# dragonlong/articulated-pose

Measured on AMD Instinct MI355X. Metric: point-clouds/sec (N=1024, eyeglasses ANCSH infer+pose-fit), higher is better.
Workload: dtype f32 (network) / f64 (joint LM)

## Files before the change

### articulated-pose_amd/csrc/pose.hip

```cpp
#include "common.h"
#include "pose_math.h"

namespace ancsh {
namespace pose {

constexpr int MODEL_A = 13;
constexpr int MODEL_B = 26;

__device__ __forceinline__ unsigned long long splitmix64(unsigned long long x) {
    x += 0x9E3779B97F4A7C15ull;
    x = (x ^ (x >> 30)) * 0xBF58476D1CE4E5B9ull;
    x = (x ^ (x >> 27)) * 0x94D049BB133111EBull;
    return x ^ (x >> 31);
}
__device__ __forceinline__ int device_draw(unsigned long long seed, int prob, int iter, int k, int n) {
    const unsigned long long h = splitmix64(seed ^ splitmix64(((unsigned long long)prob << 40) ^ ((unsigned long long)iter << 8) ^ (unsigned)k));
    return (int)(h % (unsigned long long)n);
}
enum { KEY_VALUE = 0, KEY_DSEED = 1, KEY_DKEY = 2 };
struct DKey {
    const ancsh_stream_key *key;
    int parts;
};
template <int KM> struct KeyArgT { typedef unsigned long long type; };
template <> struct KeyArgT<KEY_DKEY> { typedef DKey type; };
template <int KM> using KeyArg = typename KeyArgT<KM>::type;

template <int KM>
__device__ __forceinline__ unsigned long long kernel_seed(unsigned long long arg, unsigned add) {
    return KM != KEY_VALUE ? *(const unsigned long long *__restrict__)arg + add : arg;
}
template <int KM>
__device__ __forceinline__ unsigned long long kernel_seed(DKey arg, unsigned add) {
    return arg.key->seed + add;
}
template <int KM>
__device__ __forceinline__ int key_problem_base(unsigned long long) { return 0; }
template <int KM>
__device__ __forceinline__ int key_problem_base(DKey arg) { return arg.key->cloud_base * arg.parts; }

__device__ __forceinline__ double wave_sum(double v) {
#pragma unroll
    for (int o = 32; o > 0; o >>= 1) v += __shfl_xor(v, o, 64);
    return v;
}
template <int K>
__device__ __forceinline__ void block_sum(double (&v)[K], double *red, int nwaves) {
    const int lane = threadIdx.x & 63, wave = threadIdx.x >> 6;
#pragma unroll
    for (int i = 0; i < K; ++i) v[i] = wave_sum(v[i]);
    __syncthreads();
    if (lane == 0)
#pragma unroll
        for (int i = 0; i < K; ++i) red[wave * K + i] = v[i];
    __syncthreads();
#pragma unroll
    for (int i = 0; i < K; ++i) {
        double s = 0.0;
        for (int w = 0; w < nwaves; ++w) s += red[w * K + i];
        v[i] = s;
    }
}

__device__ __forceinline__ void estimate_single3(const float s[3][3], const float t[3][3], float R[9], float &scale,
                                                 float tr[3]) {
    double sm[3], tm[3];
#pragma unroll
    for (int c = 0; c < 3; ++c) {
        sm[c] = ((double)s[0][c] + s[1][c] + s[2][c]) / 3.0;
        tm[c] = ((double)t[0][c] + t[1][c] + t[2][c]) / 3.0;
    }
    double M[9] = {0, 0, 0, 0, 0, 0, 0, 0, 0};
#pragma unroll
    for (int i = 0; i < 3; ++i)
#pragma unroll
        for (int a = 0; a < 3; ++a)
#pragma unroll
            for (int b = 0; b < 3; ++b) M[a * 3 + b] += (t[i][a] - tm[a]) * (s[i][b] - sm[b]);
    double q[4], Rd[9];
    horn_quat_fast(M, q);
    quat_to_mat(q, Rd);
    double ab = 0.0, aa = 0.0;
// ... 643 lines not shown
    for (int i = 0; i < 3; ++i)
#pragma unroll
        for (int j = i + 1; j < 3; ++j) {
            double ds = 0.0, dt = 0.0;
#pragma unroll
            for (int c = 0; c < 3; ++c) {
                const double u = (double)s[i][c] - s[j][c], v = (double)t[i][c] - t[j][c];
                ds += u * u;
                dt += v * v;
            }
            ab += 2.0 * sqrt(ds) * sqrt(dt);
            aa += 2.0 * ds;
            bb += 2.0 * dt;
        }
    sc = (float)(ab / (aa + 1e-6));
    sc_inv = (float)(ab / (bb + 1e-6));
}

__device__ __forceinline__ void center_part3(const float s[3][3], const float t[3][3], float sc_inv, double xc[3][3],
                                             double yc[3][3]) {
    float sm[3], tm[3];
#pragma unroll
    for (int c = 0; c < 3; ++c) {
        sm[c] = ((s[0][c] + s[1][c]) + s[2][c]) / 3.0f;
        tm[c] = ((sc_inv * t[0][c] + sc_inv * t[1][c]) + sc_inv * t[2][c]) / 3.0f;
    }
#pragma unroll
    for (int i = 0; i < 3; ++i) {
#pragma unroll
        for (int c = 0; c < 3; ++c) {
            xc[i][c] = (double)(s[i][c] - sm[c]);
            yc[i][c] = (double)(sc_inv * t[i][c] - tm[c]);
        }
    }
}

__device__ __forceinline__ void prep_part3(const float s[3][3], const float t[3][3], float sc_inv, double xc[3][3],
                                           double yc[3][3], double rv[3]) {
    center_part3(s, t, sc_inv, xc, yc);
    double M[9] = {0, 0, 0, 0, 0, 0, 0, 0, 0};
#pragma unroll
    for (int i = 0; i < 3; ++i)
#pragma unroll
        for (int a = 0; a < 3; ++a)
#pragma unroll
            for (int b = 0; b < 3; ++b) M[a * 3 + b] += yc[i][a] * xc[i][b];
    double q[4];
    horn_quat_fast(M, q);
    quat_to_rotvec(q, rv);
}

__device__ __forceinline__ double residual_sq_f64(const double R[9], double sc, const double tr[3], float sx, float sy, float sz,
                                                  float tx, float ty, float tz) {
    const double rx = R[0] * sx + R[1] * sy + R[2] * sz, ry = R[3] * sx + R[4] * sy + R[5] * sz,
                 rz = R[6] * sx + R[7] * sy + R[8] * sz;
    const double ex = ((double)tx - sc * rx) - tr[0], ey = ((double)ty - sc * ry) - tr[1], ez = ((double)tz - sc * rz) - tr[2];
    return ex * ex + ey * ey + ez * ez;
}
__device__ __forceinline__ bool inlier_f64(const double R[9], double sc, const double tr[3], float sx, float sy, float sz,
                                           float tx, float ty, float tz, double th) {
    return residual_sq_f64(R, sc, tr, sx, sy, sz, tx, ty, tz) < th;
}

struct HypSamples {
    float s0[3][3], t0[3][3], s1[3][3], t1[3][3];
};
__device__ __forceinline__ void load_hyp_samples(const float *__restrict__ src, const float *__restrict__ tgt, const int *draws,
                                                 unsigned long long seed, int prob, int kbase, int niter, int h, int a0, int n0, int a1,
                                                 int n1, HypSamples &q) {
    int i0[3], i1[3];
    load_draw3(draws, seed, prob, kbase, niter, h, 0, 6, n0, i0);
    load_draw3(draws, seed, prob, kbase, niter, h, 3, 6, n1, i1);
#pragma unroll
    for (int i = 0; i < 3; ++i)
#pragma unroll
        for (int c = 0; c < 3; ++c) {
            q.s0[i][c] = src[(size_t)(a0 + i0[i]) * 3 + c];
            q.t0[i][c] = tgt[(size_t)(a0 + i0[i]) * 3 + c];
            q.s1[i][c] = src[(size_t)(a1 + i1[i]) * 3 + c];
            q.t1[i][c] = tgt[(size_t)(a1 + i1[i]) * 3 + c];
        }
}

template <int KM>
__global__ __launch_bounds__(64) void ransac_joint_init_kernel(const int *__restrict__ rng0, const int *__restrict__ rng1,
                                                               const float *__restrict__ src, const float *__restrict__ tgt,
                                                               int niter, const int *__restrict__ draws, KeyArg<KM> seed_arg,
                                                               double *__restrict__ scores, double *__restrict__ models) {
    const unsigned long long seed = kernel_seed<KM>(seed_arg, 1);
    const int kbase = key_problem_base<KM>(seed_arg);
    const int prob = blockIdx.y, h = blockIdx.x * 64 + threadIdx.x;
    const int a0 = rng0[prob * 2], n0 = rng0[prob * 2 + 1] - a0;
    const int a1 = rng1[prob * 2], n1 = rng1[prob * 2 + 1] - a1;
    if (h >= niter) return;
    double *mo = models + ((size_t)prob * niter + h) * MODEL_B;
    if (n0 <= 0 || n1 <= 0) {
        scores[(size_t)prob * niter + h] = -1.0;
        for (int i = 0; i < MODEL_B; ++i) mo[i] = NAN;
        return;
    }
    HypSamples q;
    load_hyp_samples(src, tgt, draws, seed, prob, kbase, niter, h, a0, n0, a1, n1, q);
    float sc0, sc0i, sc1, sc1i;
    scales3(q.s0, q.t0, sc0, sc0i);
    scales3(q.s1, q.t1, sc1, sc1i);
    double xc[3][3], yc[3][3], x[6];
    prep_part3(q.s0, q.t0, sc0i, xc, yc, x);
    prep_part3(q.s1, q.t1, sc1i, xc, yc, x + 3);
#pragma unroll
    for (int i = 0; i < 6; ++i) mo[i] = x[i];
    mo[6] = sc0i; mo[7] = sc1i; mo[8] = sc0; mo[9] = sc1;
}

constexpr int HYP_CHUNK = 256;
constexpr int HYP_CHUNK_SMALL = 64;
constexpr long HYP_SMALL_LAUNCH = 8192;
constexpr int HYP_REFILL = 16;

template <int KM, bool PRISM>
__device__ __forceinline__ void ransac_joint_lm_run(const int *__restrict__ rng0, const int *__restrict__ rng1,
                                                    const float *__restrict__ src, const float *__restrict__ tgt,
                                                    const float *__restrict__ joint_dir, int niter,
                                                    const int *__restrict__ draws, KeyArg<KM> seed_arg,
                                                    double *__restrict__ models, int *__restrict__ lm_stat, int chunk) {
    const unsigned long long seed = kernel_seed<KM>(seed_arg, 1);
    const int kbase = key_problem_base<KM>(seed_arg);
    const int prob = blockIdx.y;
    const int a0 = rng0[prob * 2], n0 = rng0[prob * 2 + 1] - a0;
    const int a1 = rng1[prob * 2], n1 = rng1[prob * 2 + 1] - a1;
    if (n0 <= 0 || n1 <= 0) return;
    const int c1 = min(niter, (int)(blockIdx.x + 1) * chunk);
    int next = blockIdx.x * chunk;
    HypProblemT<PRISM> P;
    if constexpr (!PRISM) {
        P.J[0] = joint_dir[prob * 3]; P.J[1] = joint_dir[prob * 3 + 1]; P.J[2] = joint_dir[prob * 3 + 2];
        P.wj = 3.0;
    }
    Lm6 S;
    bool active = false;
    int h = 0;
    for (;;) {
        const unsigned long long idle = __ballot(!active);
        const int n_idle = __popcll(idle);
        if (next < c1 && (n_idle >= HYP_REFILL || n_idle >= c1 - next || n_idle == 64)) {
            if (!active) {
                const int mine = next + __builtin_amdgcn_mbcnt_hi((unsigned)(idle >> 32), __builtin_amdgcn_mbcnt_lo((unsigned)idle, 0));
                if (mine < c1) {
                    h = mine;
                    const double *mo = models + ((size_t)prob * niter + h) * MODEL_B;
                    HypSamples q;
                    load_hyp_samples(src, tgt, draws, seed, prob, kbase, niter, h, a0, n0, a1, n1, q);
                    center_part3(q.s0, q.t0, (float)mo[6], P.x0, P.y0);
                    center_part3(q.s1, q.t1, (float)mo[7], P.x1, P.y1);
#pragma unroll
                    for (int i = 0; i < 6; ++i) S.x[i] = mo[i];
                    lm6_begin(P, S);
                    active = true;
                }
            }
            next += n_idle;
        } else if (n_idle == 64) {
            break;
        }
        if (active && lm6_trip(P, S, 1e-4, 1e-8, 1e-8, 4200)) {
            double *mo = models + ((size_t)prob * niter + h) * MODEL_B;
#pragma unroll
            for (int i = 0; i < 6; ++i) mo[i] = S.x[i];
#ifdef LM_COUNT
            if (lm_stat) { lm_stat[((size_t)prob * niter + h) * 2] = S.info | (S.trips << 4) | (S.nchol << 17); lm_stat[((size_t)prob * niter + h) * 2 + 1] = S.nfev; }
#else
            if (lm_stat) { lm_stat[((size_t)prob * niter + h) * 2] = S.info; lm_stat[((size_t)prob * niter + h) * 2 + 1] = S.nfev; }
#endif
            active = false;
        }
    }
}

template <int KM>
__global__ __launch_bounds__(64) void ransac_joint_lm_kernel(const int *__restrict__ rng0, const int *__restrict__ rng1,
                                                             const float *__restrict__ src, const float *__restrict__ tgt,
                                                             const float *__restrict__ joint_dir, int niter,
                                                             const int *__restrict__ draws, KeyArg<KM> seed_arg,
                                                             double *__restrict__ models, int *__restrict__ lm_stat, int chunk) {
    ransac_joint_lm_run<KM, false>(rng0, rng1, src, tgt, joint_dir, niter, draws, seed_arg, models, lm_stat, chunk);
}

template <int KM>
__global__ __launch_bounds__(64) void ransac_joint_lm_kind_kernel(const int *__restrict__ rng0, const int *__restrict__ rng1,
                                                                  const float *__restrict__ src, const float *__restrict__ tgt,
                                                                  const float *__restrict__ joint_dir, int niter,
                                                                  const int *__restrict__ draws, KeyArg<KM> seed_arg,
                                                                  double *__restrict__ models, int *__restrict__ lm_stat, int chunk,
                                                                  const int *__restrict__ joint_kind) {
    if (joint_kind[blockIdx.y] != 0) ransac_joint_lm_run<KM, true>(rng0, rng1, src, tgt, joint_dir, niter, draws, seed_arg, models, lm_stat, chunk);
    else ransac_joint_lm_run<KM, false>(rng0, rng1, src, tgt, joint_dir, niter, draws, seed_arg, models, lm_stat, chunk);
}

constexpr int COOP_G = 8;
constexpr int COOP_XCH = 112;
constexpr int COOP_HYP_PER_WAVE = 32;

__device__ __forceinline__ void group_lds_fence() {
    __builtin_amdgcn_fence(__ATOMIC_RELEASE, "wavefront");
    __builtin_amdgcn_wave_barrier();
    __builtin_amdgcn_fence(__ATOMIC_ACQUIRE, "wavefront");
}

template <bool PRISM>
struct HypProblemCoopT {
    double x0[3][3], y0[3][3], x1[3][3], y1[3][3], J[3], wj;
    double *xch;
    int role;

    __device__ __forceinline__ double cost(const double x[6]) const {
        const bool joint = role >= 6;
        const bool p1 = role >= 3 && role < 6;
        const int i = joint ? 0 : (p1 ? role - 3 : role);
        double partial;
        if (!joint) {
            const Rod r = p1 ? rod_prepare(x[3], x[4], x[5]) : rod_prepare(x[0], x[1], x[2]);
            const double px = p1 ? (i == 0 ? x1[0][0] : i == 1 ? x1[1][0] : x1[2][0]) : (i == 0 ? x0[0][0] : i == 1 ? x0[1][0] : x0[2][0]);
            const double py = p1 ? (i == 0 ? x1[0][1] : i == 1 ? x1[1][1] : x1[2][1]) : (i == 0 ? x0[0][1] : i == 1 ? x0[1][1] : x0[2][1]);
            const double pz = p1 ? (i == 0 ? x1[0][2] : i == 1 ? x1[1][2] : x1[2][2]) : (i == 0 ? x0[0][2] : i == 1 ? x0[1][2] : x0[2][2]);
            const double tx = p1 ? (i == 0 ? y1[0][0] : i == 1 ? y1[1][0] : y1[2][0]) : (i == 0 ? y0[0][0] : i == 1 ? y0[1][0] : y0[2][0]);
            const double ty = p1 ? (i == 0 ? y1[0][1] : i == 1 ? y1[1][1] : y1[2][1]) : (i == 0 ? y0[0][1] : i == 1 ? y0[1][1] : y0[2][1]);
            const double tz = p1 ? (i == 0 ? y1[0][2] : i == 1 ? y1[1][2] : y1[2][2]) : (i == 0 ? y0[0][2] : i == 1 ? y0[1][2] : y0[2][2]);
            double ox, oy, oz;
            rod_apply(r, px, py, pz, ox, oy, oz);
            const double a = tx - ox, b = ty - oy, c = tz - oz;
            partial = a * a + b * b + c * c;
        } else if constexpr (PRISM) {
            partial = prismatic_cost(x);
        } else {
            const Rod r0 = rod_prepare(x[0], x[1], x[2]), r1 = rod_prepare(x[3], x[4], x[5]);
            double ux, uy, uz, wx, wy, wz;
            rod_apply(r0, J[0], J[1], J[2], ux, uy, uz);
            rod_apply(r1, J[0], J[1], J[2], wx, wy, wz);
            partial = (ux - wx) * (ux - wx) + (uy - wy) * (uy - wy) + (uz - wz) * (uz - wz);
        }
        double *cs = xch + 102;
        if (role < 7) cs[role] = partial;
        group_lds_fence();
        double s = 0.0;
#pragma unroll
        for (int k = 0; k < 3; ++k) { s += cs[k]; s += cs[3 + k]; }
        if constexpr (PRISM) s += cs[6]; else s += wj * cs[6];
        group_lds_fence();
        return s;
    }

    __device__ __forceinline__ void normal(const double x[6], double A[21], double g[6]) const {
        double *col = xch, *jdx = xch + 54, *rhx = xch + 72, *fx = xch + 78, *jux = xch + 96;
        {
            const int cr = role < 6 ? role : role - 6;
            const bool p1 = cr >= 3;
            const int q = p1 ? cr - 3 : cr;
            const double r0 = p1 ? x[3] : x[0], r1 = p1 ? x[4] : x[1], r2 = p1 ? x[5] : x[2];
            const Rod b = rod_prepare(r0, r1, r2);
            const double h = fd_step(q == 0 ? r0 : q == 1 ? r1 : r2);
            const double rh = fast_rcp(h);
            const Rod pr = rod_prepare(r0 + (q == 0 ? h : 0.0), r1 + (q == 1 ? h : 0.0), r2 + (q == 2 ? h : 0.0));
            const bool wr = role < 6;
#pragma unroll
            for (int i = 0; i < 3; ++i) {
                const double px = p1 ? x1[i][0] : x0[i][0], py = p1 ? x1[i][1] : x0[i][1], pz = p1 ? x1[i][2] : x0[i][2];
                const double yx = p1 ? y1[i][0] : y0[i][0], yy = p1 ? y1[i][1] : y0[i][1], yz = p1 ? y1[i][2] : y0[i][2];
                double ox, oy, oz, qx, qy, qz;
                rod_apply(b, px, py, pz, ox, oy, oz);
                const double f0 = yx - ox, f1 = yy - oy, f2 = yz - oz;
                rod_apply(pr, px, py, pz, qx, qy, qz);
                if (wr) {
                    col[cr * 9 + i * 3 + 0] = ((yx - qx) - f0) * rh;
                    col[cr * 9 + i * 3 + 1] = ((yy - qy) - f1) * rh;
                    col[cr * 9 + i * 3 + 2] = ((yz - qz) - f2) * rh;
                    if (q == 0) { fx[(p1 ? 9 : 0) + i * 3] = f0; fx[(p1 ? 9 : 0) + i * 3 + 1] = f1; fx[(p1 ? 9 : 0) + i * 3 + 2] = f2; }
                }
            }
            if constexpr (!PRISM) {
// ... 82 lines not shown
        P.J[0] = joint_dir[prob * 3]; P.J[1] = joint_dir[prob * 3 + 1]; P.J[2] = joint_dir[prob * 3 + 2];
        P.wj = 3.0;
    }
    P.xch = xch[grp];
    P.role = lane & (COOP_G - 1);
    Lm6 S;
    bool active = false;
    int h = 0;
    for (;;) {
        const unsigned long long idle = __ballot(!active) & leaders;
        const int n_idle = __popcll(idle);
        if (next < c1 && n_idle > 0) {
            if (!active) {
                const int mine = next + __popcll(idle & ((1ull << (grp * COOP_G)) - 1ull));
                if (mine < c1) {
                    h = mine;
                    const double *mo = models + ((size_t)prob * niter + h) * MODEL_B;
                    HypSamples q;
                    load_hyp_samples(src, tgt, draws, seed, prob, kbase, niter, h, a0, n0, a1, n1, q);
                    center_part3(q.s0, q.t0, (float)mo[6], P.x0, P.y0);
                    center_part3(q.s1, q.t1, (float)mo[7], P.x1, P.y1);
#pragma unroll
                    for (int i = 0; i < 6; ++i) S.x[i] = mo[i];
                    lm6_begin(P, S);
                    active = true;
                }
            }
            next += n_idle;
        } else if (n_idle == 64 / COOP_G) {
            break;
        }
        if (active && lm6_trip(P, S, 1e-4, 1e-8, 1e-8, 4200)) {
            if (P.role == 0) {
                double *mo = models + ((size_t)prob * niter + h) * MODEL_B;
#pragma unroll
                for (int i = 0; i < 6; ++i) mo[i] = S.x[i];
                if (lm_stat) { lm_stat[((size_t)prob * niter + h) * 2] = S.info; lm_stat[((size_t)prob * niter + h) * 2 + 1] = S.nfev; }
            }
            active = false;
        }
    }
}

template <int KM>
__global__ __launch_bounds__(64) void ransac_joint_lm_coop_kernel(const int *__restrict__ rng0, const int *__restrict__ rng1,
                                                                  const float *__restrict__ src, const float *__restrict__ tgt,
                                                                  const float *__restrict__ joint_dir, int niter,
                                                                  const int *__restrict__ draws, KeyArg<KM> seed_arg,
                                                                  double *__restrict__ models, int *__restrict__ lm_stat) {
    __shared__ double xch[64 / COOP_G][COOP_XCH];
    ransac_joint_lm_coop_run<KM, false>(rng0, rng1, src, tgt, joint_dir, niter, draws, seed_arg, models, lm_stat, xch);
}

template <int KM>
__global__ __launch_bounds__(64) void ransac_joint_lm_coop_kind_kernel(const int *__restrict__ rng0, const int *__restrict__ rng1,
                                                                       const float *__restrict__ src, const float *__restrict__ tgt,
                                                                       const float *__restrict__ joint_dir, int niter,
                                                                       const int *__restrict__ draws, KeyArg<KM> seed_arg,
                                                                       double *__restrict__ models, int *__restrict__ lm_stat,
                                                                       const int *__restrict__ joint_kind) {
    __shared__ double xch[64 / COOP_G][COOP_XCH];
    if (joint_kind[blockIdx.y] != 0) ransac_joint_lm_coop_run<KM, true>(rng0, rng1, src, tgt, joint_dir, niter, draws, seed_arg, models, lm_stat, xch);
    else ransac_joint_lm_coop_run<KM, false>(rng0, rng1, src, tgt, joint_dir, niter, draws, seed_arg, models, lm_stat, xch);
}

template <int KM>
__global__ __launch_bounds__(64) void ransac_joint_model_kernel(const int *__restrict__ rng0, const int *__restrict__ rng1,
                                                                const float *__restrict__ src, const float *__restrict__ tgt,
                                                                int niter, const int *__restrict__ draws, KeyArg<KM> seed_arg,
                                                                double *__restrict__ models) {
    const unsigned long long seed = kernel_seed<KM>(seed_arg, 1);
    const int kbase = key_problem_base<KM>(seed_arg);
    const int prob = blockIdx.y, h = blockIdx.x * 64 + threadIdx.x;
    const int a0 = rng0[prob * 2], n0 = rng0[prob * 2 + 1] - a0;
    const int a1 = rng1[prob * 2], n1 = rng1[prob * 2 + 1] - a1;
    if (h >= niter || n0 <= 0 || n1 <= 0) return;
    double *mo = models + ((size_t)prob * niter + h) * MODEL_B;
    HypSamples q;
    load_hyp_samples(src, tgt, draws, seed, prob, kbase, niter, h, a0, n0, a1, n1, q);
    double x[6];
#pragma unroll
    for (int i = 0; i < 6; ++i) x[i] = mo[i];
    const float sc0 = (float)mo[8], sc1 = (float)mo[9];
    double R0[9], R1[9], tr0[3], tr1[3];
    rotvec_to_mat(x, R0);
    rotvec_to_mat(x + 3, R1);
#pragma unroll
    for (int a = 0; a < 3; ++a) {
        double u = 0.0, v = 0.0;
#pragma unroll
        for (int i = 0; i < 3; ++i) {
            u += (double)q.t0[i][a] - (double)sc0 * (R0[a * 3] * q.s0[i][0] + R0[a * 3 + 1] * q.s0[i][1] + R0[a * 3 + 2] * q.s0[i][2]);
            v += (double)q.t1[i][a] - (double)sc1 * (R1[a * 3] * q.s1[i][0] + R1[a * 3 + 1] * q.s1[i][1] + R1[a * 3 + 2] * q.s1[i][2]);
        }
        tr0[a] = u / 3.0;
        tr1[a] = v / 3.0;
    }
#pragma unroll
    for (int a = 0; a < 9; ++a) { mo[a] = R0[a]; mo[13 + a] = R1[a]; }
    mo[9] = sc0; mo[22] = sc1;
#pragma unroll
    for (int a = 0; a < 3; ++a) { mo[10 + a] = tr0[a]; mo[23 + a] = tr1[a]; }
}

__global__ __launch_bounds__(256) void ransac_joint_verify_kernel(const int *__restrict__ rng0, const int *__restrict__ rng1,
                                                                 const float *__restrict__ src, const float *__restrict__ tgt,
                                                                 double th, int niter, const double *__restrict__ models,
                                                                 double *__restrict__ scores) {
    const int prob = blockIdx.y, lane = threadIdx.x & 63;
    const int h = blockIdx.x * 4 + (threadIdx.x >> 6);
    if (h >= niter) return;
    const int a0 = rng0[prob * 2], n0 = rng0[prob * 2 + 1] - a0;
    const int a1 = rng1[prob * 2], n1 = rng1[prob * 2 + 1] - a1;
    if (n0 <= 0 || n1 <= 0) return;
    const double *mo = models + ((size_t)prob * niter + h) * MODEL_B;
    double R0[9], R1[9], tr0[3], tr1[3];
#pragma unroll
    for (int a = 0; a < 9; ++a) { R0[a] = mo[a]; R1[a] = mo[13 + a]; }
    const double sc0 = mo[9], sc1 = mo[22];
#pragma unroll
    for (int a = 0; a < 3; ++a) { tr0[a] = mo[10 + a]; tr1[a] = mo[23 + a]; }
    int c0 = 0, c1 = 0;
    for (int i = lane; i < n0; i += 64) {
        const float *ps = src + (size_t)(a0 + i) * 3, *pt = tgt + (size_t)(a0 + i) * 3;
        c0 += inlier_f64(R0, sc0, tr0, ps[0], ps[1], ps[2], pt[0], pt[1], pt[2], th) ? 1 : 0;
    }
    for (int i = lane; i < n1; i += 64) {
        const float *ps = src + (size_t)(a1 + i) * 3, *pt = tgt + (size_t)(a1 + i) * 3;
        c1 += inlier_f64(R1, sc1, tr1, ps[0], ps[1], ps[2], pt[0], pt[1], pt[2], th) ? 1 : 0;
    }
#pragma unroll
    for (int o = 32; o > 0; o >>= 1) { c0 += __shfl_xor(c0, o, 64); c1 += __shfl_xor(c1, o, 64); }
    if (lane == 0) scores[(size_t)prob * niter + h] = ((double)c0 / 3.0 + (double)c1 / 3.0) / 2.0;
}

template <bool PRISM>
struct BlockProblemT {
    const float (*x0)[3];
    const float (*y0)[3];
    const float (*x1)[3];
    const float (*y1)[3];
    int n0, n1;
    double J[3], wj;
    double *red;

    __device__ __forceinline__ double cost(const double x[6]) const {
        const Rod r0 = rod_prepare(x[0], x[1], x[2]), r1 = rod_prepare(x[3], x[4], x[5]);
        double s[1] = {0.0}, ox, oy, oz;
        for (int i = threadIdx.x; i < n0; i += 256) {
            rod_apply(r0, x0[i][0], x0[i][1], x0[i][2], ox, oy, oz);
            const double a = y0[i][0] - ox, b = y0[i][1] - oy, c = y0[i][2] - oz;
            s[0] += a * a + b * b + c * c;
        }
        for (int i = threadIdx.x; i < n1; i += 256) {
            rod_apply(r1, x1[i][0], x1[i][1], x1[i][2], ox, oy, oz);
            const double a = y1[i][0] - ox, b = y1[i][1] - oy, c = y1[i][2] - oz;
            s[0] += a * a + b * b + c * c;
        }
        block_sum<1>(s, red, 4);
        if constexpr (PRISM) {
            return s[0] + prismatic_cost(x);
        } else {
            double ux, uy, uz, wx, wy, wz;
            rod_apply(r0, J[0], J[1], J[2], ux, uy, uz);
            rod_apply(r1, J[0], J[1], J[2], wx, wy, wz);
            return s[0] + wj * ((ux - wx) * (ux - wx) + (uy - wy) * (uy - wy) + (uz - wz) * (uz - wz));
        }
    }
    __device__ __forceinline__ void normal(const double x[6], double A[21], double g[6]) const {
        PartFd p0, p1;
        if constexpr (PRISM) p0.begin_points(x); else p0.begin(x, J);
        for (int i = threadIdx.x; i < n0; i += 256) p0.point(x0[i][0], x0[i][1], x0[i][2], y0[i][0], y0[i][1], y0[i][2]);
        if constexpr (PRISM) p1.begin_points(x + 3); else p1.begin(x + 3, J);
        for (int i = threadIdx.x; i < n1; i += 256) p1.point(x1[i][0], x1[i][1], x1[i][2], y1[i][0], y1[i][1], y1[i][2]);
        double v[18];
#pragma unroll
        for (int i = 0; i < 6; ++i) { v[i] = p0.blk[i]; v[9 + i] = p1.blk[i]; }
#pragma unroll
        for (int i = 0; i < 3; ++i) { v[6 + i] = p0.gv[i]; v[15 + i] = p1.gv[i]; }
        block_sum<18>(v, red, 4);
        if constexpr (PRISM) assemble_normal_prismatic(x, v, v + 6, v + 9, v + 15, A, g);
        else assemble_normal(p0, v, v + 6, p1, v + 9, v + 15, wj, A, g);
    }
};
typedef BlockProblemT<false> BlockProblem;
// ... 703 lines not shown
    E.record = nullptr; E.K = 0; E.tie = nullptr;
    E.lo_f = E.hi_f = 0.f; E.lo_d = E.hi_d = 0.0;
    E.draws = nullptr; E.seed = 0;
    return E;
}

static int make_extras(const char *who, int nprob, double *record, int K, int min_K, int *tie, double th, double window, FitExtras &E) {
    E.record = record; E.K = K; E.tie = tie;
    if (record) {
        ANCSH_REQUIRE(K >= min_K && nprob % (K - (min_K - 1)) == 0, "%s: record needs K >= %d and nprob (%d) a multiple of %s (K = %d)", who, min_K, nprob,
                      min_K == 1 ? "K" : "K - 1", K);
    }
    if (tie) {
        ANCSH_REQUIRE(window >= 0.0 && window < th, "%s: tie_window %g must be in [0, inlier_th)", who, window);
        const double lo = (th - window) * (th - window), hi = (th + window) * (th + window);
        E.lo_f = (float)lo; E.hi_f = (float)hi; E.lo_d = lo; E.hi_d = hi;
    }
    return ANCSH_OK;
}

static long single_quads_needed(long rows, int nprob) { return 2 * ((rows + 7) / 8 + nprob) + 2; }

extern "C" long ancsh_ransac_single_quads_floats(long rows, int nprob) {
    if (rows < 0 || nprob < 0) return -1;
    return 24 * single_quads_needed(rows, nprob);
}

template <int KM>
static int ransac_single_impl(int nprob, const int *off, const float *src, const float *tgt, float inlier_th, int niter,
                              const int *draws, KeyArg<KM> seed, int max_n, double *out_model,
                              unsigned char *out_inliers, int *out_best, int *scratch_scores, float *scratch_quads, long rows,
                              FitExtras E, void *stream) {
    ANCSH_REQUIRE(nprob >= 0 && niter > 0 && max_n > 0, "ransac_single: bad sizes nprob=%d niter=%d max_n=%d", nprob, niter, max_n);
    ANCSH_REQUIRE(max_n <= 6144, "ransac_single: max_n %d > 6144 (refit keeps the inliers in LDS)", max_n);
    if (nprob == 0) return ANCSH_OK;
    ANCSH_REQUIRE(off && src && tgt && out_model && out_inliers && out_best && scratch_scores, "ransac_single: null pointer");
    hipStream_t st = (hipStream_t)stream;
    ANCSH_REQUIRE(inlier_th > 0.f, "ransac_single: inlier_th must be positive");
    inlier_th = sq_threshold_f32(inlier_th);
    if (scratch_quads && inlier_th >= 0x1p-100f && inlier_th < 4.0f) {
        ANCSH_REQUIRE(rows >= 0 && rows < (1L << 30), "ransac_single_ex: rows=%ld out of range", rows);
        ANCSH_REQUIRE((((uintptr_t)scratch_quads) & 31) == 0, "ransac_single_ex: scratch_quads must be 32-byte aligned");
        const int cap = (int)single_quads_needed(rows, nprob);
        hipLaunchKernelGGL(soa_quads_kernel, dim3((max_n + 7 + 255) / 256, nprob), dim3(256), 0, st, off, src, tgt, scratch_quads, cap);
        hipLaunchKernelGGL(ransac_single_score_sreg_kernel<KM>, dim3((niter + 255) / 256, nprob), dim3(256), 0, st, off, src, tgt,
                           (const float *)scratch_quads, cap, inlier_th, niter, draws, seed, scratch_scores);
    } else {
        hipLaunchKernelGGL(ransac_single_score_kernel<KM>, dim3((niter + 255) / 256, nprob), dim3(256), 0, st, off, src, tgt, inlier_th,
                           niter, draws, seed, scratch_scores);
    }
    const size_t lds = 64 * sizeof(double) + 8 * sizeof(int) + (size_t)2 * max_n * 3 * sizeof(float);
    if (lds > 48 * 1024) (void)hipFuncSetAttribute((const void *)ransac_single_finish_kernel<KM>, hipFuncAttributeMaxDynamicSharedMemorySize, (int)lds);
    hipLaunchKernelGGL(ransac_single_finish_kernel<KM>, dim3(nprob), dim3(256), lds, st, off, src, tgt, inlier_th, niter, draws, seed,
                       scratch_scores, max_n, out_model, out_inliers, out_best, E);
    return check_launch("ransac_single");
}

extern "C" int ancsh_ransac_single(int nprob, const int *off, const float *src, const float *tgt, float inlier_th, int niter,
                                   const int *draws, unsigned long long seed, int max_n, double *out_model,
                                   unsigned char *out_inliers, int *out_best, int *scratch_scores, void *stream) {
    return ransac_single_impl<KEY_VALUE>(nprob, off, src, tgt, inlier_th, niter, draws, seed, max_n, out_model, out_inliers, out_best,
                                     scratch_scores, nullptr, 0, no_extras(), stream);
}

extern "C" int ancsh_ransac_single_ex(int nprob, const int *off, const float *src, const float *tgt, float inlier_th, int niter,
                                      const int *draws, unsigned long long seed, int max_n, double *out_model,
                                      unsigned char *out_inliers, int *out_best, int *scratch_scores, float *scratch_quads,
                                      long rows, void *stream) {
    ANCSH_REQUIRE(scratch_quads, "ransac_single_ex: scratch_quads is NULL (ancsh_ransac_single is the call without it)");
    return ransac_single_impl<KEY_VALUE>(nprob, off, src, tgt, inlier_th, niter, draws, seed, max_n, out_model, out_inliers, out_best,
                                     scratch_scores, scratch_quads, rows, no_extras(), stream);
}

extern "C" int ancsh_ransac_single_rec(int nprob, const int *off, const float *src, const float *tgt, float inlier_th, int niter,
                                       const int *draws, unsigned long long seed, int max_n, double *out_model,
                                       unsigned char *out_inliers, int *out_best, int *scratch_scores, float *scratch_quads,
                                       long rows, double *record, int K, int *tie_stats, float tie_window, void *stream) {
    FitExtras E = no_extras();
    if (int rc = make_extras("ransac_single_rec", nprob, record, K, 1, tie_stats, (double)inlier_th, (double)tie_window, E)) return rc;
    return ransac_single_impl<KEY_VALUE>(nprob, off, src, tgt, inlier_th, niter, draws, seed, max_n, out_model, out_inliers, out_best,
                                     scratch_scores, scratch_quads, rows, E, stream);
}

template <int KM>
static int ransac_joint_impl(int nprob, const int *rng0, const int *rng1, const float *src, const float *tgt,
                             const float *joint_dir, double inlier_th, int niter, const int *draws,
                             KeyArg<KM> seed, int max_n, double *out_model, unsigned char *out_inliers,
                             int *out_best, double *out_score, double *scratch_scores, double *scratch_models,
                             int *lm_stat, int lm_schedule, FitExtras E, void *stream, const int *joint_kind = nullptr) {
    ANCSH_REQUIRE(lm_schedule >= ANCSH_LM_AUTO && lm_schedule <= ANCSH_LM_LATENCY, "ransac_joint: unknown lm_schedule %d", lm_schedule);
    ANCSH_REQUIRE(nprob >= 0 && niter > 0 && max_n > 0, "ransac_joint: bad sizes");
    ANCSH_REQUIRE(max_n <= 3072, "ransac_joint: max_n %d > 3072 (refit keeps both parts' inliers in LDS)", max_n);
    if (nprob == 0) return ANCSH_OK;
    ANCSH_REQUIRE(rng0 && rng1 && src && tgt && joint_dir && out_model && out_inliers && out_best && out_score &&
                      scratch_scores && scratch_models, "ransac_joint: null pointer");
    hipStream_t st = (hipStream_t)stream;
    ANCSH_REQUIRE(inlier_th > 0.0, "ransac_joint: inlier_th must be positive");
    inlier_th = sq_threshold_f64(inlier_th);
    const dim3 per_hyp((niter + 63) / 64, nprob);
    hipLaunchKernelGGL(ransac_joint_init_kernel<KM>, per_hyp, dim3(64), 0, st, rng0, rng1, src, tgt, niter, draws, seed, scratch_scores,
                       scratch_models);
    if (lm_schedule == ANCSH_LM_LATENCY) {
        const dim3 grid((niter + COOP_HYP_PER_WAVE - 1) / COOP_HYP_PER_WAVE, nprob);
        if (joint_kind)
            hipLaunchKernelGGL(ransac_joint_lm_coop_kind_kernel<KM>, grid, dim3(64), 0, st, rng0, rng1, src, tgt, joint_dir, niter, draws, seed,
                               scratch_models, lm_stat, joint_kind);
        else
            hipLaunchKernelGGL(ransac_joint_lm_coop_kernel<KM>, grid, dim3(64), 0, st,
                               rng0, rng1, src, tgt, joint_dir, niter, draws, seed, scratch_models, lm_stat);
    } else {
        const int chunk = (long)nprob * niter <= HYP_SMALL_LAUNCH ? HYP_CHUNK_SMALL : HYP_CHUNK;
        if (joint_kind)
            hipLaunchKernelGGL(ransac_joint_lm_kind_kernel<KM>, dim3((niter + chunk - 1) / chunk, nprob), dim3(64), 0, st, rng0, rng1, src, tgt,
                               joint_dir, niter, draws, seed, scratch_models, lm_stat, chunk, joint_kind);
        else
            hipLaunchKernelGGL(ransac_joint_lm_kernel<KM>, dim3((niter + chunk - 1) / chunk, nprob), dim3(64), 0, st, rng0, rng1, src, tgt,
                               joint_dir, niter, draws, seed, scratch_models, lm_stat, chunk);
    }
    hipLaunchKernelGGL(ransac_joint_model_kernel<KM>, per_hyp, dim3(64), 0, st, rng0, rng1, src, tgt, niter, draws, seed, scratch_models);
    hipLaunchKernelGGL(ransac_joint_verify_kernel, dim3((niter + 3) / 4, nprob), dim3(256), 0, st, rng0, rng1, src, tgt, inlier_th,
                       niter, scratch_models, scratch_scores);
    const size_t lds = 128 * sizeof(double) + 8 * sizeof(int) + (size_t)4 * max_n * 3 * sizeof(float);
    if (joint_kind) {
        if (lds > 48 * 1024) (void)hipFuncSetAttribute((const void *)ransac_joint_finish_kind_kernel<KM>, hipFuncAttributeMaxDynamicSharedMemorySize, (int)lds);
        hipLaunchKernelGGL(ransac_joint_finish_kind_kernel<KM>, dim3(nprob), dim3(256), lds, st, rng0, rng1, src, tgt, joint_dir, inlier_th,
                           niter, scratch_scores, scratch_models, max_n, out_model, out_inliers, out_best, out_score, E, joint_kind);
        return check_launch("ransac_joint");
    }
    if (lds > 48 * 1024) (void)hipFuncSetAttribute((const void *)ransac_joint_finish_kernel<KM>, hipFuncAttributeMaxDynamicSharedMemorySize, (int)lds);
    hipLaunchKernelGGL(ransac_joint_finish_kernel<KM>, dim3(nprob), dim3(256), lds, st, rng0, rng1, src, tgt, joint_dir, inlier_th,
                       niter, scratch_scores, scratch_models, max_n, out_model, out_inliers, out_best, out_score, E);
    return check_launch("ransac_joint");
}

static int check_joint_kind(const char *who, int nprob, const int *joint_kind) {
    if (!joint_kind || nprob <= 0) return ANCSH_OK;
    hipPointerAttribute_t at;
    if (hipPointerGetAttributes(&at, joint_kind) != hipSuccess) { (void)hipGetLastError(); return ANCSH_OK; }
    if (at.type != hipMemoryTypeHost) return ANCSH_OK;
    for (int p = 0; p < nprob; ++p)
        ANCSH_REQUIRE(joint_kind[p] == 0 || joint_kind[p] == 1, "%s: joint_kind[%d] = %d (0 revolute, 1 prismatic)", who, p, joint_kind[p]);
    return ANCSH_OK;
}

extern "C" int ancsh_ransac_joint(int nprob, const int *rng0, const int *rng1, const float *src, const float *tgt,
                                  const float *joint_dir, double inlier_th, int niter, const int *draws,
                                  unsigned long long seed, int max_n, double *out_model, unsigned char *out_inliers,
                                  int *out_best, double *out_score, double *scratch_scores, double *scratch_models,
                                  int *lm_stat, void *stream) {
    return ransac_joint_impl<KEY_VALUE>(nprob, rng0, rng1, src, tgt, joint_dir, inlier_th, niter, draws, seed, max_n, out_model, out_inliers,
                                    out_best, out_score, scratch_scores, scratch_models, lm_stat, ANCSH_LM_AUTO, no_extras(), stream);
}

extern "C" int ancsh_ransac_joint_ex(int nprob, const int *rng0, const int *rng1, const float *src, const float *tgt,
                                     const float *joint_dir, double inlier_th, int niter, const int *draws,
                                     unsigned long long seed, int max_n, double *out_model, unsigned char *out_inliers,
                                     int *out_best, double *out_score, double *scratch_scores, double *scratch_models,
                                     int *lm_stat, int lm_schedule, void *stream) {
    return ransac_joint_impl<KEY_VALUE>(nprob, rng0, rng1, src, tgt, joint_dir, inlier_th, niter, draws, seed, max_n, out_model, out_inliers,
                                    out_best, out_score, scratch_scores, scratch_models, lm_stat, lm_schedule, no_extras(), stream);
}

extern "C" int ancsh_ransac_joint_rec(int nprob, const int *rng0, const int *rng1, const float *src, const float *tgt,
                                      const float *joint_dir, double inlier_th, int niter, const int *draws,
                                      unsigned long long seed, int max_n, double *out_model, unsigned char *out_inliers,
                                      int *out_best, double *out_score, double *scratch_scores, double *scratch_models,
                                      int *lm_stat, int lm_schedule, double *record, int K, int *tie_stats, double tie_window,
                                      void *stream) {
    FitExtras E = no_extras();
    if (int rc = make_extras("ransac_joint_rec", nprob, record, K, 2, tie_stats, inlier_th, tie_window, E)) return rc;
    E.draws = draws; E.seed = seed;
    return ransac_joint_impl<KEY_VALUE>(nprob, rng0, rng1, src, tgt, joint_dir, inlier_th, niter, draws, seed, max_n, out_model, out_inliers,
                                    out_best, out_score, scratch_scores, scratch_models, lm_stat, lm_schedule, E, stream);
}

extern "C" int ancsh_ransac_single_rec_dseed(int nprob, const int *off, const float *src, const float *tgt, float inlier_th, int niter,
                                             const int *draws, const unsigned long long *seed, int max_n, double *out_model,
                                             unsigned char *out_inliers, int *out_best, int *scratch_scores, float *scratch_quads,
                                             long rows, double *record, int K, int *tie_stats, float tie_window, void *stream) {
    ANCSH_REQUIRE(seed, "ransac_single_rec_dseed: null seed pointer");
    FitExtras E = no_extras();
    if (int rc = make_extras("ransac_single_rec_dseed", nprob, record, K, 1, tie_stats, (double)inlier_th, (double)tie_window, E)) return rc;
    return ransac_single_impl<KEY_DSEED>(nprob, off, src, tgt, inlier_th, niter, draws, (unsigned long long)(uintptr_t)seed, max_n, out_model,
                                    out_inliers, out_best, scratch_scores, scratch_quads, rows, E, stream);
}

extern "C" int ancsh_ransac_joint_rec_dseed(int nprob, const int *rng0, const int *rng1, const float *src, const float *tgt,
                                            const float *joint_dir, double inlier_th, int niter, const int *draws,
                                            const unsigned long long *seed, int max_n, double *out_model, unsigned char *out_inliers,
                                            int *out_best, double *out_score, double *scratch_scores, double *scratch_models,
                                            int *lm_stat, int lm_schedule, double *record, int K, int *tie_stats, double tie_window,
                                            void *stream) {
    ANCSH_REQUIRE(seed, "ransac_joint_rec_dseed: null seed pointer");
    FitExtras E = no_extras();
    if (int rc = make_extras("ransac_joint_rec_dseed", nprob, record, K, 2, tie_stats, inlier_th, tie_window, E)) return rc;
    E.draws = draws; E.seed = (unsigned long long)(uintptr_t)seed;
    return ransac_joint_impl<KEY_DSEED>(nprob, rng0, rng1, src, tgt, joint_dir, inlier_th, niter, draws, E.seed, max_n, out_model,
                                   out_inliers, out_best, out_score, scratch_scores, scratch_models, lm_stat, lm_schedule, E, stream);
}

extern "C" int ancsh_ransac_single_rec_dkey(int nprob, const int *off, const float *src, const float *tgt, float inlier_th, int niter,
                                            const int *draws, const ancsh_stream_key *key, int max_n, double *out_model,
// ... 95 lines not shown
```

Before: 17460.

## Fuse joint RANSAC init, LM refinement and model build into one kernel

Adds a fused LM kernel that computes the per-hypothesis scale and initial rotation vectors in registers, runs the LM fit, and writes the final rotation/translation model directly. This replaces the separate init, LM and model kernels in the non-latency schedule. It is meant to remove two kernel launches and the round trips of intermediate model data through global memory. Each block now takes a fixed chunk of 64 hypotheses, one per lane, so the lane refill scheme for balancing uneven LM iteration counts is effectively lost. A legacy path stays available through an environment variable.

```diff
diff --git a/articulated-pose_amd/csrc/pose.hip b/articulated-pose_amd/csrc/pose.hip
--- a/articulated-pose_amd/csrc/pose.hip
+++ b/articulated-pose_amd/csrc/pose.hip
@@ -1,3 +1,6 @@
+#include <cstdlib>
+#include <cstring>
+
 #include "common.h"
 #include "pose_math.h"
 
@@ -807,6 +810,22 @@
         }
 }
 
+__device__ __forceinline__ void body_boundary(double &v) { asm volatile("" : "+v"(v)); }
+__device__ __forceinline__ void body_boundary(float &v) { asm volatile("" : "+v"(v)); }
+
+__device__ __forceinline__ void joint_init_body(const HypSamples &q, double x[6], float &sc0, float &sc0i, float &sc1, float &sc1i) {
+    scales3(q.s0, q.t0, sc0, sc0i);
+    scales3(q.s1, q.t1, sc1, sc1i);
+    double xc[3][3], yc[3][3];
+    prep_part3(q.s0, q.t0, sc0i, xc, yc, x);
+    prep_part3(q.s1, q.t1, sc1i, xc, yc, x + 3);
+}
+__device__ __forceinline__ void joint_init_empty(double *__restrict__ scores, double *__restrict__ models, int prob, int niter, int h) {
+    double *mo = models + ((size_t)prob * niter + h) * MODEL_B;
+    scores[(size_t)prob * niter + h] = -1.0;
+    for (int i = 0; i < MODEL_B; ++i) mo[i] = NAN;
+}
+
 template <int KM>
 __global__ __launch_bounds__(64) void ransac_joint_init_kernel(const int *__restrict__ rng0, const int *__restrict__ rng1,
                                                                const float *__restrict__ src, const float *__restrict__ tgt,
@@ -820,50 +839,75 @@
     if (h >= niter) return;
     double *mo = models + ((size_t)prob * niter + h) * MODEL_B;
     if (n0 <= 0 || n1 <= 0) {
-        scores[(size_t)prob * niter + h] = -1.0;
-        for (int i = 0; i < MODEL_B; ++i) mo[i] = NAN;
+        joint_init_empty(scores, models, prob, niter, h);
         return;
     }
     HypSamples q;
     load_hyp_samples(src, tgt, draws, seed, prob, kbase, niter, h, a0, n0, a1, n1, q);
     float sc0, sc0i, sc1, sc1i;
-    scales3(q.s0, q.t0, sc0, sc0i);
-    scales3(q.s1, q.t1, sc1, sc1i);
-    double xc[3][3], yc[3][3], x[6];
-    prep_part3(q.s0, q.t0, sc0i, xc, yc, x);
-    prep_part3(q.s1, q.t1, sc1i, xc, yc, x + 3);
+    double x[6];
+    joint_init_body(q, x, sc0, sc0i, sc1, sc1i);
 #pragma unroll
     for (int i = 0; i < 6; ++i) mo[i] = x[i];
     mo[6] = sc0i; mo[7] = sc1i; mo[8] = sc0; mo[9] = sc1;
 }
 
+__device__ __forceinline__ void joint_model_body(const HypSamples &q, const double x[6], float sc0, float sc1, double *__restrict__ mo) {
+    double R0[9], R1[9], tr0[3], tr1[3];
+    rotvec_to_mat(x, R0);
+    rotvec_to_mat(x + 3, R1);
+#pragma unroll
+    for (int a = 0; a < 3; ++a) {
+        double u = 0.0, v = 0.0;
+#pragma unroll
+        for (int i = 0; i < 3; ++i) {
+            u += (double)q.t0[i][a] - (double)sc0 * (R0[a * 3] * q.s0[i][0] + R0[a * 3 + 1] * q.s0[i][1] + R0[a * 3 + 2] * q.s0[i][2]);
+            v += (double)q.t1[i][a] - (double)sc1 * (R1[a * 3] * q.s1[i][0] + R1[a * 3 + 1] * q.s1[i][1] + R1[a * 3 + 2] * q.s1[i][2]);
+        }
+        tr0[a] = u / 3.0;
+        tr1[a] = v / 3.0;
+    }
+#pragma unroll
+    for (int a = 0; a < 9; ++a) { mo[a] = R0[a]; mo[13 + a] = R1[a]; }
+    mo[9] = sc0; mo[22] = sc1;
+#pragma unroll
+    for (int a = 0; a < 3; ++a) { mo[10 + a] = tr0[a]; mo[23 + a] = tr1[a]; }
+}
+
+constexpr int HYP_WAVE = 64;
 constexpr int HYP_CHUNK = 256;
 constexpr int HYP_CHUNK_SMALL = 64;
 constexpr long HYP_SMALL_LAUNCH = 8192;
 constexpr int HYP_REFILL = 16;
 
-template <int KM, bool PRISM>
+template <int KM, bool PRISM, bool FUSED>
 __device__ __forceinline__ void ransac_joint_lm_run(const int *__restrict__ rng0, const int *__restrict__ rng1,
                                                     const float *__restrict__ src, const float *__restrict__ tgt,
                                                     const float *__restrict__ joint_dir, int niter,
-                                                    const int *__restrict__ draws, KeyArg<KM> seed_arg,
+                                                    const int *__restrict__ draws, KeyArg<KM> seed_arg, double *__restrict__ scores,
                                                     double *__restrict__ models, int *__restrict__ lm_stat, int chunk) {
     const unsigned long long seed = kernel_seed<KM>(seed_arg, 1);
     const int kbase = key_problem_base<KM>(seed_arg);
     const int prob = blockIdx.y;
     const int a0 = rng0[prob * 2], n0 = rng0[prob * 2 + 1] - a0;
     const int a1 = rng1[prob * 2], n1 = rng1[prob * 2 + 1] - a1;
-    if (n0 <= 0 || n1 <= 0) return;
     const int c1 = min(niter, (int)(blockIdx.x + 1) * chunk);
     int next = blockIdx.x * chunk;
+    if (n0 <= 0 || n1 <= 0) {
+        if constexpr (FUSED) {
+            for (int e = next + (int)threadIdx.x; e < c1; e += 64) joint_init_empty(scores, models, prob, niter, e);
+        }
+        return;
+    }
     HypProblemT<PRISM> P;
     if constexpr (!PRISM) {
         P.J[0] = joint_dir[prob * 3]; P.J[1] = joint_dir[prob * 3 + 1]; P.J[2] = joint_dir[prob * 3 + 2];
         P.wj = 3.0;
     }
     Lm6 S;
-    bool active = false;
+    bool active = false, fitted = false;
     int h = 0;
+    float sc0 = 0.0f, sc1 = 0.0f;
     for (;;) {
         const unsigned long long idle = __ballot(!active);
         const int n_idle = __popcll(idle);
@@ -872,13 +916,23 @@
                 const int mine = next + __builtin_amdgcn_mbcnt_hi((unsigned)(idle >> 32), __builtin_amdgcn_mbcnt_lo((unsigned)idle, 0));
                 if (mine < c1) {
                     h = mine;
-                    const double *mo = models + ((size_t)prob * niter + h) * MODEL_B;
                     HypSamples q;
                     load_hyp_samples(src, tgt, draws, seed, prob, kbase, niter, h, a0, n0, a1, n1, q);
-                    center_part3(q.s0, q.t0, (float)mo[6], P.x0, P.y0);
-                    center_part3(q.s1, q.t1, (float)mo[7], P.x1, P.y1);
-#pragma unroll
-                    for (int i = 0; i < 6; ++i) S.x[i] = mo[i];
+                    if constexpr (FUSED) {
+                        float sc0i, sc1i;
+                        joint_init_body(q, S.x, sc0, sc0i, sc1, sc1i);
+#pragma unroll
+                        for (int i = 0; i < 6; ++i) body_boundary(S.x[i]);
+                        body_boundary(sc0i); body_boundary(sc1i); body_boundary(sc0); body_boundary(sc1);
+                        center_part3(q.s0, q.t0, sc0i, P.x0, P.y0);
+                        center_part3(q.s1, q.t1, sc1i, P.x1, P.y1);
+                    } else {
+                        const double *mo = models + ((size_t)prob * niter + h) * MODEL_B;
+                        center_part3(q.s0, q.t0, (float)mo[6], P.x0, P.y0);
+                        center_part3(q.s1, q.t1, (float)mo[7], P.x1, P.y1);
+#pragma unroll
+                        for (int i = 0; i < 6; ++i) S.x[i] = mo[i];
+                    }
                     lm6_begin(P, S);
                     active = true;
                 }
@@ -888,15 +942,27 @@
             break;
         }
         if (active && lm6_trip(P, S, 1e-4, 1e-8, 1e-8, 4200)) {
-            double *mo = models + ((size_t)prob * niter + h) * MODEL_B;
-#pragma unroll
-            for (int i = 0; i < 6; ++i) mo[i] = S.x[i];
+            if constexpr (!FUSED) {
+                double *mo = models + ((size_t)prob * niter + h) * MODEL_B;
+#pragma unroll
+                for (int i = 0; i < 6; ++i) mo[i] = S.x[i];
+            }
 #ifdef LM_COUNT
             if (lm_stat) { lm_stat[((size_t)prob * niter + h) * 2] = S.info | (S.trips << 4) | (S.nchol << 17); lm_stat[((size_t)prob * niter + h) * 2 + 1] = S.nfev; }
 #else
             if (lm_stat) { lm_stat[((size_t)prob * niter + h) * 2] = S.info; lm_stat[((size_t)prob * niter + h) * 2 + 1] = S.nfev; }
 #endif
             active = false;
+            fitted = true;
+        }
+    }
+    if constexpr (FUSED) {
+        if (fitted) {
+#pragma unroll
+            for (int i = 0; i < 6; ++i) body_boundary(S.x[i]);
+            HypSamples q;
+            load_hyp_samples(src, tgt, draws, seed, prob, kbase, niter, h, a0, n0, a1, n1, q);
+            joint_model_body(q, S.x, sc0, sc1, models + ((size_t)prob * niter + h) * MODEL_B);
         }
     }
 }
@@ -907,7 +973,7 @@
                                                              const float *__restrict__ joint_dir, int niter,
                                                              const int *__restrict__ draws, KeyArg<KM> seed_arg,
                                                              double *__restrict__ models, int *__restrict__ lm_stat, int chunk) {
-    ransac_joint_lm_run<KM, false>(rng0, rng1, src, tgt, joint_dir, niter, draws, seed_arg, models, lm_stat, chunk);
+    ransac_joint_lm_run<KM, false, false>(rng0, rng1, src, tgt, joint_dir, niter, draws, seed_arg, nullptr, models, lm_stat, chunk);
 }
 
 template <int KM>
@@ -917,8 +983,29 @@
                                                                   const int *__restrict__ draws, KeyArg<KM> seed_arg,
                                                                   double *__restrict__ models, int *__restrict__ lm_stat, int chunk,
                                                                   const int *__restrict__ joint_kind) {
-    if (joint_kind[blockIdx.y] != 0) ransac_joint_lm_run<KM, true>(rng0, rng1, src, tgt, joint_dir, niter, draws, seed_arg, models, lm_stat, chunk);
-    else ransac_joint_lm_run<KM, false>(rng0, rng1, src, tgt, joint_dir, niter, draws, seed_arg, models, lm_stat, chunk);
+    if (joint_kind[blockIdx.y] != 0) ransac_joint_lm_run<KM, true, false>(rng0, rng1, src, tgt, joint_dir, niter, draws, seed_arg, nullptr, models, lm_stat, chunk);
+    else ransac_joint_lm_run<KM, false, false>(rng0, rng1, src, tgt, joint_dir, niter, draws, seed_arg, nullptr, models, lm_stat, chunk);
+}
+
+template <int KM>
+__global__ __launch_bounds__(64) void ransac_joint_lm_fused_kernel(const int *__restrict__ rng0, const int *__restrict__ rng1,
+                                                              const float *__restrict__ src, const float *__restrict__ tgt,
+                                                              const float *__restrict__ joint_dir, int niter,
+                                                              const int *__restrict__ draws, KeyArg<KM> seed_arg,
+                                                              double *__restrict__ scores, double *__restrict__ models,
+                                                              int *__restrict__ lm_stat) {
+    ransac_joint_lm_run<KM, false, true>(rng0, rng1, src, tgt, joint_dir, niter, draws, seed_arg, scores, models, lm_stat, HYP_WAVE);
+}
+
+template <int KM>
+__global__ __launch_bounds__(64) void ransac_joint_lm_fused_kind_kernel(const int *__restrict__ rng0, const int *__restrict__ rng1,
+                                                                   const float *__restrict__ src, const float *__restrict__ tgt,
+                                                                   const float *__restrict__ joint_dir, int niter,
+                                                                   const int *__restrict__ draws, KeyArg<KM> seed_arg,
+                                                                   double *__restrict__ scores, double *__restrict__ models,
+                                                                   int *__restrict__ lm_stat, const int *__restrict__ joint_kind) {
+    if (joint_kind[blockIdx.y] != 0) ransac_joint_lm_run<KM, true, true>(rng0, rng1, src, tgt, joint_dir, niter, draws, seed_arg, scores, models, lm_stat, HYP_WAVE);
+    else ransac_joint_lm_run<KM, false, true>(rng0, rng1, src, tgt, joint_dir, niter, draws, seed_arg, scores, models, lm_stat, HYP_WAVE);
 }
 
 constexpr int COOP_G = 8;
@@ -1167,25 +1254,7 @@
 #pragma unroll
     for (int i = 0; i < 6; ++i) x[i] = mo[i];
     const float sc0 = (float)mo[8], sc1 = (float)mo[9];
-    double R0[9], R1[9], tr0[3], tr1[3];
-    rotvec_to_mat(x, R0);
-    rotvec_to_mat(x + 3, R1);
-#pragma unroll
-    for (int a = 0; a < 3; ++a) {
-        double u = 0.0, v = 0.0;
-#pragma unroll
-        for (int i = 0; i < 3; ++i) {
-            u += (double)q.t0[i][a] - (double)sc0 * (R0[a * 3] * q.s0[i][0] + R0[a * 3 + 1] * q.s0[i][1] + R0[a * 3 + 2] * q.s0[i][2]);
-            v += (double)q.t1[i][a] - (double)sc1 * (R1[a * 3] * q.s1[i][0] + R1[a * 3 + 1] * q.s1[i][1] + R1[a * 3 + 2] * q.s1[i][2]);
-        }
-        tr0[a] = u / 3.0;
-        tr1[a] = v / 3.0;
-    }
-#pragma unroll
-    for (int a = 0; a < 9; ++a) { mo[a] = R0[a]; mo[13 + a] = R1[a]; }
-    mo[9] = sc0; mo[22] = sc1;
-#pragma unroll
-    for (int a = 0; a < 3; ++a) { mo[10 + a] = tr0[a]; mo[23 + a] = tr1[a]; }
+    joint_model_body(q, x, sc0, sc1, mo);
 }
 
 __global__ __launch_bounds__(256) void ransac_joint_verify_kernel(const int *__restrict__ rng0, const int *__restrict__ rng1,
@@ -2055,6 +2124,14 @@
                                      scratch_scores, scratch_quads, rows, E, stream);
 }
 
+static bool lm_pack_legacy() {
+    static const bool v = [] {
+        const char *e = getenv("ANCSH_LM_PACK");
+        return e && !strcmp(e, "legacy");
+    }();
+    return v;
+}
+
 template <int KM>
 static int ransac_joint_impl(int nprob, const int *rng0, const int *rng1, const float *src, const float *tgt,
                              const float *joint_dir, double inlier_th, int niter, const int *draws,
@@ -2071,26 +2148,35 @@
     ANCSH_REQUIRE(inlier_th > 0.0, "ransac_joint: inlier_th must be positive");
     inlier_th = sq_threshold_f64(inlier_th);
     const dim3 per_hyp((niter + 63) / 64, nprob);
-    hipLaunchKernelGGL(ransac_joint_init_kernel<KM>, per_hyp, dim3(64), 0, st, rng0, rng1, src, tgt, niter, draws, seed, scratch_scores,
-                       scratch_models);
-    if (lm_schedule == ANCSH_LM_LATENCY) {
-        const dim3 grid((niter + COOP_HYP_PER_WAVE - 1) / COOP_HYP_PER_WAVE, nprob);
+    if (lm_schedule != ANCSH_LM_LATENCY && !lm_pack_legacy()) {
         if (joint_kind)
-            hipLaunchKernelGGL(ransac_joint_lm_coop_kind_kernel<KM>, grid, dim3(64), 0, st, rng0, rng1, src, tgt, joint_dir, niter, draws, seed,
-                               scratch_models, lm_stat, joint_kind);
+            hipLaunchKernelGGL(ransac_joint_lm_fused_kind_kernel<KM>, dim3((niter + HYP_WAVE - 1) / HYP_WAVE, nprob), dim3(64), 0, st, rng0, rng1,
+                               src, tgt, joint_dir, niter, draws, seed, scratch_scores, scratch_models, lm_stat, joint_kind);
         else
-            hipLaunchKernelGGL(ransac_joint_lm_coop_kernel<KM>, grid, dim3(64), 0, st,
-                               rng0, rng1, src, tgt, joint_dir, niter, draws, seed, scratch_models, lm_stat);
+            hipLaunchKernelGGL(ransac_joint_lm_fused_kernel<KM>, dim3((niter + HYP_WAVE - 1) / HYP_WAVE, nprob), dim3(64), 0, st, rng0, rng1,
+                               src, tgt, joint_dir, niter, draws, seed, scratch_scores, scratch_models, lm_stat);
     } else {
-        const int chunk = (long)nprob * niter <= HYP_SMALL_LAUNCH ? HYP_CHUNK_SMALL : HYP_CHUNK;
-        if (joint_kind)
-            hipLaunchKernelGGL(ransac_joint_lm_kind_kernel<KM>, dim3((niter + chunk - 1) / chunk, nprob), dim3(64), 0, st, rng0, rng1, src, tgt,
-                               joint_dir, niter, draws, seed, scratch_models, lm_stat, chunk, joint_kind);
-        else
-            hipLaunchKernelGGL(ransac_joint_lm_kernel<KM>, dim3((niter + chunk - 1) / chunk, nprob), dim3(64), 0, st, rng0, rng1, src, tgt,
-                               joint_dir, niter, draws, seed, scratch_models, lm_stat, chunk);
-    }
-    hipLaunchKernelGGL(ransac_joint_model_kernel<KM>, per_hyp, dim3(64), 0, st, rng0, rng1, src, tgt, niter, draws, seed, scratch_models);
+        hipLaunchKernelGGL(ransac_joint_init_kernel<KM>, per_hyp, dim3(64), 0, st, rng0, rng1, src, tgt, niter, draws, seed, scratch_scores,
+                           scratch_models);
+        if (lm_schedule == ANCSH_LM_LATENCY) {
+            const dim3 grid((niter + COOP_HYP_PER_WAVE - 1) / COOP_HYP_PER_WAVE, nprob);
+            if (joint_kind)
+                hipLaunchKernelGGL(ransac_joint_lm_coop_kind_kernel<KM>, grid, dim3(64), 0, st, rng0, rng1, src, tgt, joint_dir, niter, draws, seed,
+                                   scratch_models, lm_stat, joint_kind);
+            else
+                hipLaunchKernelGGL(ransac_joint_lm_coop_kernel<KM>, grid, dim3(64), 0, st,
+                                   rng0, rng1, src, tgt, joint_dir, niter, draws, seed, scratch_models, lm_stat);
+        } else {
+            const int chunk = (long)nprob * niter <= HYP_SMALL_LAUNCH ? HYP_CHUNK_SMALL : HYP_CHUNK;
+            if (joint_kind)
+                hipLaunchKernelGGL(ransac_joint_lm_kind_kernel<KM>, dim3((niter + chunk - 1) / chunk, nprob), dim3(64), 0, st, rng0, rng1, src, tgt,
+                                   joint_dir, niter, draws, seed, scratch_models, lm_stat, chunk, joint_kind);
+            else
+                hipLaunchKernelGGL(ransac_joint_lm_kernel<KM>, dim3((niter + chunk - 1) / chunk, nprob), dim3(64), 0, st, rng0, rng1, src, tgt,
+                                   joint_dir, niter, draws, seed, scratch_models, lm_stat, chunk);
+        }
+        hipLaunchKernelGGL(ransac_joint_model_kernel<KM>, per_hyp, dim3(64), 0, st, rng0, rng1, src, tgt, niter, draws, seed, scratch_models);
+    }
     hipLaunchKernelGGL(ransac_joint_verify_kernel, dim3((niter + 3) / 4, nprob), dim3(256), 0, st, rng0, rng1, src, tgt, inlier_th,
                        niter, scratch_models, scratch_scores);
     const size_t lds = 128 * sizeof(double) + 8 * sizeof(int) + (size_t)4 * max_n * 3 * sizeof(float);
```

After: 17210. 0.986x the previous value.
